# chinaxuyongtao/x264-vs2008

Hardware: AMD Instinct MI355X
Metric: encoded frames/sec, 1080p, preset=medium's flag set with the encoder's own lookahead and rate control (--crf 23 --b-adapt 1, hex, subme 7 RD, trellis 1, psy-rd, aq-mode 1, CABAC payload on the GPU); 1/2/4/8 MI355X (bit-exact) (higher is better)
Workload: dtype u8

## Files before the change

### x264_vs2008_amd/csrc/slice_kernel.h

```cpp
#pragma once
#include <cstddef>
#include <cstring>
#include "me_exact.h"
#include "intra_pred.h"
#include "frame_internal.h"
#include "mb_vocab.h"
#include "trellis_wave.h"
#include "cabac_price.h"

using namespace x264hip;

#define SW_MAX_REFS 8
#define SW_SPIN_LIMIT (1 << 21)
#define SW_MB_BYTES_MAX 8192
#define FD 32
#define FDY (2 * FD)
#define FDU (19 * FD)
#define FDV (19 * FD + 16)

enum { NB_LEFT = 1, NB_TOP = 2, NB_TOPRIGHT = 4, NB_TOPLEFT = 8 };

struct SwRefs {
    const u8 *y[SW_MAX_REFS][4];
    const u8 *u[SW_MAX_REFS], *v[SW_MAX_REFS];
    int ref_bits[SW_MAX_REFS], poc_delta[SW_MAX_REFS], l0_inv_ref_poc[SW_MAX_REFS];
    const u8 *y1[4], *u1, *v1;
    int biw[SW_MAX_REFS];
    int dsf[SW_MAX_REFS], map_col[SW_MAX_REFS];
};
struct SwArgs {
    int mb_w, mb_h, sy, sc, batch, batch_pad;
    int chain;
    size_t bs_y, bs_c;
    int slice_type, qp, qpc, lambda, chroma_skip_thresh, n_refs;
    int l0_n_ref0;
    int me_method, me_range, subme, chroma_me, fast_pskip, dct_decimate, cabac, mv_range;
    int flags_inter, mixed_refs;
    int flags_intra;
    int transform8x8;
    const u16 *q4mf, *q4bias, *q8mf, *q8bias;
    const int *dq4, *dq8;
    const i16 *cost_mv;
    int cost_center;
    const i16 *lowres0, *lowres1;
    const u8 *fy, *fu, *fv;
    u8 *dy, *du, *dv;
    const signed char *l0_type, *l0_ref;
    const i16 *l0_mv;
    signed char *mb_type, *partition, *sub_partition, *ref, *i4mode, *i16mode, *chroma_mode, *qp_out, *t8;
    i16 *mv, *mvr, *cbp;
    u8 *nnz;
    i16 *luma, *luma_dc, *chroma_dc, *chroma_ac;
    int *cost_intra, *cost_inter, *cost_alt;
    int *progress, *abort_flag;
    int *abort_total;
    int spin_limit;
    long long *prof;
    int nr;
    int lossless;
    u32 *nr_sum, *nr_count;
    const u16 *nr_offset;
};

struct SwQp { int qp, qpc, lambda, lambda2, skip_thresh; };

struct SwLds {
    __attribute__((aligned(16))) u8 fe[384];
    u8 fd[27 * FD];
    i16 coef[16][16];
    i16 ccoef[8][16];
    int score[16], cscore[8];
    i16 cdc[8], cdcout[8], dc16[16];
    int keep8, cmode[2], nzdc16;
    i16 lv_y[256], lv_dc[16], lv_cdc[8], lv_cac[128];
    u8 nnz[32];
    i16 mvc[9][2];
    i16 left_mvr[SW_MAX_REFS][2];
    signed char i4c[48];
    u8 e4[16], edge8[40];
    __attribute__((aligned(4))) u8 pt4[48];
    __attribute__((aligned(4))) u8 pt8[80];
    u32 p4lut[48], p8lut[192];
    u16 nr_off4[16], nr_off8[64];
    __attribute__((aligned(16))) u8 patch[MX_PATCH_BYTES];
    u8 i4_fdec[256], i8_fdec[256], i4_nnz[16], i8_nnz[16];
    i16 lv_y8[256];
    i16 t8[256];
    signed char left_i4[4];
    signed char pred4[16], pred8[4];
    i16 l0mvc[SW_MAX_REFS][5][2];
    i16 mv4[16][2];
    signed char ref8[4];
    i16 left_mv4[4][2];
    signed char left_r8[2];
    u16 q8mf[2][64], q8bias[2][64];
    int q8dq[2][64];
    u16 qmf[4][16], qbias[4][16];
    int qdq[4][16];
    i16 costl[2 * MX_COST_LDS + 2];
};

struct SwRd {
    int on;
    int mbrd, trellis, psy_rd;
    int write, cabac_init_idc, i_frame, i_frame_stride;
    int aq, qp_min, qp_max, chroma_qp_offset;
    float f_qpm;
    int psy_trellis;
    const float *aq_offset;
    const i16 *cost_mv_all;
    const int *unq4, *unq8;
    u8 *payload; int payload_cap;
    u32 psy_carry_lo;
    int *payload_len, *mb_bits;
    i16 *mvd;
    i16 *mv1, *mvr1, *mvd1;
    signed char *ref1;
    union {
        u8 *skipbp;
        u8 *mb_carry;
    };
    const signed char *col_type, *col_ref;
    const i16 *col_mv;
    int direct_temporal;
    u32 psy_carry_hi;
    int *direct_score;
    i16 *stale;
};
static_assert(offsetof(SwRd, psy_carry_lo) == offsetof(SwRd, payload_cap) + 4 && offsetof(SwRd, payload_len) == offsetof(SwRd, psy_carry_lo) + 4 &&
              offsetof(SwRd, psy_carry_hi) == offsetof(SwRd, direct_temporal) + 4 && offsetof(SwRd, direct_score) == offsetof(SwRd, psy_carry_hi) + 4,
              "the two halves of the psy-trellis carry's address fill padding: the kernel argument of every other kernel keeps its layout");
struct SwLdsB {
    signed char cref1[48], cskip[48];
    i16 cmv1[48][2], cmvd1[48][2];
    signed char dref[2][4], sub[4];
    i16 dmv[2][16][2];
    i16 mv4_1[16][2];
    signed char ref8_1[4];
    i16 left_mv4_1[4][2], left_mvd1[4][2], left_mvr1[2];
    signed char left_r8_1[2];
    u8 left_skipbp;
    i16 stale[6];
    int me[2][9][6];
    int cost8direct[4];
};
struct SwLdsRdB;
static __device__ const u8 c_bidir_dirs[32] = {149, 21, 101, 69, 89, 81, 86, 84, 165, 5, 105, 65, 90, 80, 150, 20, 153, 17, 102, 68, 133, 37, 97, 73, 88, 82, 22, 148, 145, 25, 100, 70};
struct SwLdsRd {
    u8 cabac[460], cabac_tmp[460];
    signed char cref[48], sub[4];
    i16 cmv[48][2], cmvd[48][2];
    u8 nz_l[4], nz_t[4], nz_lc[2][2], nz_tc[2][2];
    i16 i4_dct[256], i8_dct[256];
    int fenc_satd[16], fenc_sa8d[4];
    int unq4[4][16], unq8[2][64];
    i16 left_mvd[4][2];
    u8 left_nz[8];
    u8 zz2[4], zz4[16], zz8[64];
    int w4z[16], w8z[64];
    u8 zero16[16];
    int tmp_i[4];
    TdWave tw;
};
struct SwLdsNone { int unused; };
struct SwLdsRdB { SwLdsRd r; SwLdsB b; };
struct SwLdsRf { int i16dir[8], cdir[4], i8dir[12][4]; u8 pels[16]; };
struct SwLdsRdF { SwLdsRd r; SwLdsRf f; };
struct MbSynDev {
    int slice_type, type, partition, i16mode, chroma_mode, cbp_luma, cbp_chroma, t8, qp, n_ref, pps_t8, t8_allowed;
    int type_left, type_top, cbp_left, cbp_top, cpm_left, cpm_top, nb_t8, last_qp, last_dqp, prev_coded;
    signed char *sub, *i4c, *cref;
    i16 (*cmv)[2], (*cmvd)[2];
    int n_ref1;
    signed char *cref1, *cskip;
    i16 (*cmv1)[2], (*cmvd1)[2];
    u8 *nnz, *nz_l, *nz_t;
    u8 (*nz_lc)[2], (*nz_tc)[2];
    i16 (*lv4)[16], (*lv8)[64], *lv_dc, (*lv_cdc)[4], (*lv_cac)[16];
};
struct SwTq { static constexpr bool PSY = false; int on; SwLdsRd *r; };
enum { SW_PSY_OWN = 0, SW_PSY_ZERO = 1, SW_PSY_KEPT = 2 };
struct SwTqPsy { static constexpr bool PSY = true; int on; SwLdsRd *r; int psy, src4, src8; i16 *kept; };
__device__ __forceinline__ void sw_tq_set_psy(SwTq &, int, int, i16 *) {}
__device__ __forceinline__ void sw_tq_set_psy(SwTqPsy &tq, int psy, int src, i16 *kept) { tq.psy = psy; tq.src4 = tq.src8 = src; tq.kept = kept; }
__device__ __forceinline__ i16 *sw_psy_carry(const SwRd &rd, int bz)
{
    const unsigned long long p = ((unsigned long long)rd.psy_carry_hi << 32) | rd.psy_carry_lo;
    return p ? (i16 *)p + (size_t)bz * 512 : nullptr;
}
static __device__ const int d_w4z[16] = {800, 320, 320, 800, 128, 800, 320, 320, 320, 320, 128, 800, 128, 320, 320, 128};
static __device__ const u8 d_zz4[16] = {0, 4, 1, 2, 5, 8, 12, 9, 6, 3, 7, 10, 13, 14, 11, 15};
static __device__ const u8 d_zz2[4] = {0, 1, 2, 3};
static __device__ const u16 d_w8k[6] = {256, 201, 656, 227, 410, 363};
static __device__ const u8 d_w8cls[16] = {0, 3, 4, 3, 3, 1, 5, 1, 4, 5, 2, 5, 3, 1, 5, 1};
__device__ __forceinline__ int sw_w8z(int pos) { const int r = c_scan8[0][pos]; return d_w8k[d_w8cls[((r >> 1) & 12) | (r & 3)]]; }
struct SwW8 { __device__ __forceinline__ int operator[](int pos) const { return sw_w8z(pos); } };

#define WAVE_SYNC() do { __builtin_amdgcn_fence(__ATOMIC_RELEASE, "workgroup", "local"); __builtin_amdgcn_wave_barrier(); \
                         __builtin_amdgcn_fence(__ATOMIC_ACQUIRE, "workgroup", "local"); } while (0)

__device__ __forceinline__ void sw_blk_xy(int k, int &x, int &y)
{
    x = ((k >> 2) & 1) * 8 + (k & 1) * 4;
    y = (k >> 3) * 8 + ((k >> 1) & 1) * 4;
}
__device__ __forceinline__ int sw_decimate(const i16 *lv, int n)
{
    int i = n - 1, score = 0;
    while (i >= 0 && lv[i] == 0) i--;
    while (i >= 0) {
        if ((unsigned)(lv[i--] + 1) > 2u) return 9;
        int run = 0;
        while (i >= 0 && lv[i] == 0) { i--; run++; }
        score += c_decimate4[run];
    }
    return score;
}
__device__ __forceinline__ int sw_ue_size(int v) { return v == 0 ? 1 : v < 3 ? 3 : 5; }

__device__ __forceinline__ void sw_mc16(SwLds &s, const SwRefs &refs, const SwArgs &a, int ri, int mvx, int mvy, ptrdiff_t oy, ptrdiff_t oc,
                                        size_t by, size_t bc, int lane, bool do_chroma)
{
    {
        const int r = lane >> 2, x = (lane & 3) * 4;
        const int qx = mvx & 3, qy = mvy & 3, idx = qy * 4 + qx;
        const ptrdiff_t base = oy + (ptrdiff_t)((mvy >> 2) + r) * a.sy + (mvx >> 2) + x + (ptrdiff_t)by;
        const u8 *pa = refs.y[ri][c_qpel_a[idx]] + base + (qy == 3) * a.sy;
        const u8 *pb = refs.y[ri][c_qpel_b[idx]] + base + (qx == 3);
#pragma unroll
        for (int i = 0; i < 4; i++)
            s.fd[FDY + r * FD + x + i] = (idx & 5) ? (u8)(((int)pa[i] + (int)pb[i] + 1) >> 1) : pa[i];
    }
    if (do_chroma) {
        const int cx = lane & 7, cy = lane >> 3;
        const int dx = mvx & 7, dyy = mvy & 7;
        const int ca = (8 - dx) * (8 - dyy), cb = dx * (8 - dyy), cc = (8 - dx) * dyy, cd = dx * dyy;
        const ptrdiff_t cbase = oc + (ptrdiff_t)((mvy >> 3) + cy) * a.sc + (mvx >> 3) + cx + (ptrdiff_t)bc;
        const u8 *pu = refs.u[ri] + cbase, *pv = refs.v[ri] + cbase;
        s.fd[FDU + cy * FD + cx] = (u8)((ca * pu[0] + cb * pu[1] + cc * pu[a.sc] + cd * pu[a.sc + 1] + 32) >> 6);
        s.fd[FDV + cy * FD + cx] = (u8)((ca * pv[0] + cb * pv[1] + cc * pv[a.sc] + cd * pv[a.sc + 1] + 32) >> 6);
    }
}

__device__ __forceinline__ void sw_mc_parts(SwLds &s, const SwRefs &refs, const SwArgs &a, ptrdiff_t oy, ptrdiff_t oc, size_t by, size_t bc, int lane,
                                            bool clip = false, int mbx = 0, int mby = 0)
// ... 1094 lines not shown
```

### x264_vs2008_amd/csrc/slice_sweep_body.h

```cpp
    static_assert(!CH || RD, "the chain table belongs to the raster variant");
    constexpr bool SUB8 = RF && !LL;
    SwRd rd_l;
    if constexpr (CH) {
        typedef const __attribute__((address_space(4))) SwDesc *desc_p;
        const desc_p d = (desc_p)(uintptr_t)tab + blockIdx.x;
        typedef const __attribute__((address_space(4))) u32 *word_p;
        static_assert(sizeof(SwArgs) % 4 == 0 && sizeof(SwRd) % 4 == 0 && alignof(SwDesc) >= 4, "copied by dwords");
        const word_p wa = (word_p)&d->a, wr = (word_p)&d->r;
#pragma unroll
        for (unsigned i = 0; i < sizeof(SwArgs) / 4; i++) ((u32 *)&a)[i] = wa[i];
#pragma unroll
        for (unsigned i = 0; i < sizeof(SwRd) / 4; i++) ((u32 *)&rd_l)[i] = wr[i];
    }
    const SwRd &rd = CH ? rd_l : rd_k;
    const SwRefs &refs = CH ? tab[blockIdx.x].t : refs_k;
    if constexpr (CH && !BS) __builtin_amdgcn_s_setprio(3);
    static_assert(!BS || RD, "B slices run in the raster variant");
    static_assert(!TD || BS, "temporal direct prediction is a B-slice matter");
    static_assert(!RF || (RD && !BS), "the RD refinement is built for the raster variant's I / P kernel");
#undef IS_SKIP_T
#define IS_SKIP_T(t) (BS ? ((t) == T_P_SKIP || (t) == T_B_SKIP) : (t) == T_P_SKIP)
    __builtin_assume(a.lossless == (int)LL);
    __shared__ SwLds s;
    __shared__ typename std::conditional<BS, SwLdsRdB, typename std::conditional<RF, SwLdsRdF, typename std::conditional<RD, SwLdsRd, SwLdsNone>::type>::type>::type sr_;
// ... 491 lines not shown
                } else
                cbp_luma = t8 ? sw_encode_inter_luma8(s, a, Q, tq, lane, &nr_acc8, nr_on) : sw_encode_inter_luma(s, a, Q, tq, lane, &nr_acc4, nr_on);
                cbp_chroma = sw_encode_chroma(s, a, Q, tq, 1, lane);
                if (type == T_P_L0 && part == D_16x16 && !(cbp_luma | cbp_chroma) && mvx == pskx && mvy == psky && ref == 0) type = T_P_SKIP;
                if (BS && type == T_B_DIRECT && !(cbp_luma | cbp_chroma)) type = T_B_SKIP;
            }
        };

        int fenc_satd_sum = 0, fenc_sa8d_sum = 0;
        auto cache_fenc_satd = [&]() {
            if constexpr (PT && !BS) { if (rd.trellis == 2 && a.subme == 6) sw_psy_before_trials(s, tq, a.transform8x8, lane); }
            if (!rd.psy_rd) return;
            int v4 = 0, v8 = 0;
            if (lane < 16) {
                const u8 *fe = s.fe + (lane >> 2) * 64 + (lane & 3) * 4;
                int sad = 0;
#pragma unroll
                for (int j = 0; j < 4; j++)
#pragma unroll
                    for (int i = 0; i < 4; i++) sad += fe[j * 16 + i];
                v4 = satd_4x4(sr.zero16, 0, fe, 16) - (sad >> 1);
            } else if (lane < 20) {
                const int b = lane - 16;
                const u8 *fe = s.fe + (b >> 1) * 128 + (b & 1) * 8;
                int sad = 0;
                for (int j = 0; j < 8; j++)
#pragma unroll
                    for (int i = 0; i < 8; i++) sad += fe[j * 16 + i];
                v8 = ((sa8d_8x8_raw(sr.zero16, 0, fe, 16) + 2) >> 2) - (sad >> 2);
            }
            fenc_satd_sum = wave_sum(v4); fenc_sa8d_sum = wave_sum(v8);
            if constexpr (RF) {
                if (lane < 16) sr.fenc_satd[lane] = v4; else if (lane < 20) sr.fenc_sa8d[lane - 16] = v8;
                WAVE_SYNC();
            }
        };
        auto ssd_mb = [&]() -> int {
            int acc = 0;
            {
                const int r = lane >> 2, x = (lane & 3) * 4, cx = lane & 7, cy = lane >> 3;
#pragma unroll
                for (int i = 0; i < 4; i++) { const int d = (int)s.fe[r * 16 + x + i] - (int)s.fd[FDY + r * FD + x + i]; acc += d * d; }
                const int du = (int)s.fe[256 + cy * 8 + cx] - (int)s.fd[FDU + cy * FD + cx], dv = (int)s.fe[320 + cy * 8 + cx] - (int)s.fd[FDV + cy * FD + cx];
                acc += du * du + dv * dv;
            }
            int ssd = wave_sum(acc);
            if (rd.psy_rd) {
                unsigned long long h = 0;
                if (lane < 4) h = hadamard_ac_8x8(s.fd + FDY + (lane >> 1) * 8 * FD + (lane & 1) * 8, FD);
                const u32 lo = (u32)h, hi = (u32)(h >> 32);
                unsigned long long sum = 0;
#pragma unroll
                for (int k = 0; k < 4; k++) sum += ((unsigned long long)(u32)__builtin_amdgcn_readlane((int)hi, k) << 32) + (u32)__builtin_amdgcn_readlane((int)lo, k);
                const int s4 = (int)((u32)sum >> 1), s8 = (int)(sum >> 34);
                const int satd = (iabs(s4 - fenc_satd_sum) + iabs(s8 - fenc_sa8d_sum)) >> 1;
                ssd += (satd * rd.psy_rd * Q.lambda + 128) >> 8;
            }
            return ssd;
        };
        auto syn_prepare = [&]() {
            if (is_p && lane < 16) {
                const int k = 12 + (lane & 3) + 8 * (lane >> 2);
                sr.cref[k] = s.ref8[(lane >> 3) * 2 + ((lane & 3) >> 1)]; sr.cmv[k][0] = s.mv4[lane][0]; sr.cmv[k][1] = s.mv4[lane][1];
            }
            if (lane < 4) sr.sub[lane] = (signed char)sub_t_mb;
            WAVE_SYNC();
        };
        auto make_syn = [&]() -> MbSynDev {
            MbSynDev y;
            y.slice_type = a.slice_type; y.type = type; y.partition = part; y.i16mode = pred16; y.chroma_mode = predc;
            y.cbp_luma = cbp_luma; y.cbp_chroma = cbp_chroma; y.t8 = t8; y.qp = Q.qp; y.n_ref = a.n_refs; y.pps_t8 = a.transform8x8;
            y.t8_allowed = a.transform8x8 && (type == T_P_L0 || (type == T_P_8x8 && __ballot(lane < 4 && sub_t_mb != D_L0_8x8) == 0));
            if constexpr (BS) y.t8_allowed = a.transform8x8 && type >= T_B_DIRECT && type <= T_B_8x8;
            y.type_left = left_type == T_I_8x8 ? T_I_4x4 : left_type; y.type_top = type_top == T_I_8x8 ? T_I_4x4 : type_top; y.cbp_left = left_cbp; y.cbp_top = cbp_top; y.cpm_left = left_cpm; y.cpm_top = cpm_top;
            y.nb_t8 = (left_type >= 0 && left_t8) + (type_top >= 0 && t8_top);
            y.last_qp = last_qp; y.last_dqp = last_dqp; y.prev_coded = prev_coded;
            y.sub = sr.sub; y.i4c = s.i4c; y.cref = sr.cref; y.cmv = sr.cmv; y.cmvd = sr.cmvd;
            y.n_ref1 = 0; y.cref1 = nullptr; y.cskip = nullptr; y.cmv1 = nullptr; y.cmvd1 = nullptr;
            if constexpr (BS) { y.n_ref1 = 1; y.sub = sb.sub; y.cref1 = sb.cref1; y.cskip = sb.cskip; y.cmv1 = sb.cmv1; y.cmvd1 = sb.cmvd1; }
            y.nnz = s.nnz; y.nz_l = sr.nz_l; y.nz_t = sr.nz_t; y.nz_lc = sr.nz_lc; y.nz_tc = sr.nz_tc;
            y.lv4 = (i16 (*)[16])s.lv_y; y.lv8 = (i16 (*)[64])s.lv_y8; y.lv_dc = s.lv_dc; y.lv_cdc = (i16 (*)[4])s.lv_cdc; y.lv_cac = (i16 (*)[16])s.lv_cac;
            return y;
        };
        auto price_mb = [&]() -> int {
            syn_prepare();
            for (int k = lane; k < 460; k += 64) sr.cabac_tmp[k] = sr.cabac[k];
            const MbSynDev y0 = make_syn();
            const CpMasks km = cp_masks([&](int q) -> cp_u64 { return __ballot(cp_mask_lane(y0, q, lane)); });
            WAVE_SYNC();
            if (lane == 0) {
                DCabac tcb = {0, 0x1FE, -1, 0, nullptr, 0};
                MbSynDev y = y0;
                cp_macroblock(tcb, sr.cabac_tmp, y, km);
                sr.tmp_i[0] = tcb.f8;
            }
            WAVE_SYNC();
            return UNI(sr.tmp_i[0]);
        };
        (void)cache_fenc_satd; (void)ssd_mb; (void)price_mb;
        const int satd_pcm = RD && !rd.psy_rd && mbrd ? (int)(((unsigned long long)(386 * 8) * (u32)Q.lambda2 + 128) >> 8) : MX_COST_MAX;

        if constexpr (BS) {
#include "slice_b_flow.h"
        } else
        if (!RD && !is_p) {
          {
            analyse_intra(MX_COST_MAX);
            type = T_I_16x16;
            int i_cost = satd_i16;
            if (satd_i4 < i_cost) { i_cost = satd_i4; type = T_I_4x4; }
            if (satd_i8 < i_cost) { i_cost = satd_i8; type = T_I_8x8; }
          }
        } else {
            int ra = left_ref, ax = left_mvx, ay = left_mvy;
            int rb = -2, bx = 0, byv = 0, rc = -2, cx = 0, cy = 0;
            if (is_p && (nb & NB_TOP)) { const int o = mb - a.mb_w; rb = UNI(a.ref[o * 4 + 2]); bx = UNI(a.mv[(o * 16 + 12) * 2]); byv = UNI(a.mv[(o * 16 + 12) * 2 + 1]); }
            if (!is_p) {}
            else if (nb & NB_TOPRIGHT) { const int o = mb - a.mb_w + 1; rc = UNI(a.ref[o * 4 + 2]); cx = UNI(a.mv[(o * 16 + 12) * 2]); cy = UNI(a.mv[(o * 16 + 12) * 2 + 1]); }
            else if (nb & NB_TOPLEFT) { const int o = mb - a.mb_w - 1; rc = UNI(a.ref[o * 4 + 3]); cx = UNI(a.mv[(o * 16 + 15) * 2]); cy = UNI(a.mv[(o * 16 + 15) * 2 + 1]); }
            int cref_v = -2, cmvx_v = 0, cmvy_v = 0, pme_v = 0;
            int sub_mx = 0, sub_my = 0, sub_cost = 0, sub_px = 0, sub_py = 0, sub_t = D_L0_8x8;
            int sub_cst = MX_COST_MAX;
            (void)sub_cst;
            if (is_p && (RD || (a.flags_inter & 0x10))) {
                if ((nb & NB_TOP) && lane >= 4 && lane < 8) {
                    const int o = mb - a.mb_w, k = lane - 4;
                    cref_v = a.ref[o * 4 + 2 + (k >> 1)]; cmvx_v = a.mv[(o * 16 + 12 + k) * 2]; cmvy_v = a.mv[(o * 16 + 12 + k) * 2 + 1];
                }
                if ((nb & NB_TOPLEFT) && lane == 3) {
                    const int o = mb - a.mb_w - 1;
                    cref_v = a.ref[o * 4 + 3]; cmvx_v = a.mv[(o * 16 + 15) * 2]; cmvy_v = a.mv[(o * 16 + 15) * 2 + 1];
                }
                if ((nb & NB_TOPRIGHT) && lane == 8) {
                    const int o = mb - a.mb_w + 1;
                    cref_v = a.ref[o * 4 + 2]; cmvx_v = a.mv[(o * 16 + 12) * 2]; cmvy_v = a.mv[(o * 16 + 12) * 2 + 1];
                }
                if ((nb & NB_LEFT) && lane >= 11 && lane < 36 && ((lane - 11) & 7) == 0) {
                    const int i = (lane - 11) >> 3;
                    cref_v = s.left_r8[i >> 1]; cmvx_v = s.left_mv4[i][0]; cmvy_v = s.left_mv4[i][1];
                }
            }
            if constexpr (RD) { if (is_p && lane == 30) { cref_v = st0r; cmvx_v = st0x; cmvy_v = st0y; } }
            if constexpr (RD) {
                if (is_p) {
                    if (lane < 48) { sr.cref[lane] = (signed char)cref_v; sr.cmv[lane][0] = (i16)cmvx_v; sr.cmv[lane][1] = (i16)cmvy_v; }
                    WAVE_SYNC();
                }
            }
            auto predict16 = [&](int i_ref, int &px, int &py) {
                const int cnt = (ra == i_ref) + (rb == i_ref) + (rc == i_ref);
                if (cnt > 1) { px = mb_median(ax, bx, cx); py = mb_median(ay, byv, cy); }
                else if (cnt == 1) { if (ra == i_ref) { px = ax; py = ay; } else if (rb == i_ref) { px = bx; py = byv; } else { px = cx; py = cy; } }
                else if (rb == -2 && rc == -2 && ra != -2) { px = ax; py = ay; }
                else { px = mb_median(ax, bx, cx); py = mb_median(ay, byv, cy); }
            };
            if (ra == -2 || rb == -2 || !(ra | ax | ay) || !(rb | bx | byv)) { pskx = 0; psky = 0; }
            else predict16(0, pskx, psky);

            int b_skip = 0, try_pskip = 0;
            if (is_p && a.fast_pskip) {
                if (a.subme >= 3) try_pskip = 1;
                else if (left_type == T_P_SKIP || type_top == T_P_SKIP || type_topleft == T_P_SKIP || type_topright == T_P_SKIP) {
                    b_skip = sw_probe_pskip(s, refs, a, Q, pskx, psky, mbx, mby, oy, oc, by_, bc_, lane);
                    skip_mc = b_skip;
                }
            }
            if (b_skip) type = T_P_SKIP;
            else {
                const MeLimits L = me_limits(mbx, mby, a.mb_w, a.mb_h, a.mv_range);
                MxCtx c;
                c.fe = (MX_LDS(u32))s.fe; c.fe_u = (MX_LDS(u8))(s.fe + 256); c.fe_v = (MX_LDS(u8))(s.fe + 320); c.sy = a.sy; c.sc = a.sc; c.lane = lane; c.set_block(16, 16, 0, 0);
                c.cost_g = (MX_GLB(i16))cost_g;
                c.cost_l = (MX_LDS(i16))s.costl; c.has_cost_l = true; c.patch = (MX_LDS(u8))s.patch; c.has_patch = true; c.patch_on = false;
                int thresh = 0x7fffffff, best = 0x7fffffff, bmvpx = 0, bmvpy = 0;
                bool early_skip = false;
                for (int r = 0; r < (is_p ? a.n_refs : 0); r++) {
// ... 468 lines not shown
                                    continue;
                                } else {
                                    tq.on = rd.trellis != 0;
                                    if (rd.trellis == 1 || a.nr) skip_intra = 0;
                                }
                            } else if (step == 11) {
                                if constexpr (RF) {
#include "slice_refine.h"
                                }
                            } else {
                                fin = true;
                                tq.on = rd.trellis != 0;
                                if (rd.trellis == 1 || a.nr) skip_intra = 0;
                            }
                            if ((!fin || mbrd) && !IS_INTRA_T(type)) update_cache_p();
                            const int t8_bak = t8;
                            PROF(6);
                            if (!(fin && type == T_I_PCM)) encode_mb(fin ? 1 : 0);
                            else psy_after_analysis();
                            if (fin) { encoded = true; break; }
                            PROF(0);
                            int c = ssd_mb();
                            if (type == T_P_SKIP) c += (Q.lambda2 + 128) >> 8;
                            else {
                                const int f8 = price_mb();
                                c += (int)(((unsigned long long)(u32)f8 * (u32)Q.lambda2 + 32768) >> 16);
                            }
                            t8 = t8_bak;
                            PROF(7);
                            if (step == 0) { rd16 = c; if (type == T_P_SKIP) rd_skip = true; }
                            else if (step == 2) rd16 = c;
                            else if (step == 3) c16x8 = c;
                            else if (step == 4) c8x16 = c;
                            else if (step == 5) c8x8 = c;
                            else if (step == 6) {
                                if (i_cost >= c) {
                                    if (i_cost > 0) satd_inter = (int)((long long)satd_inter * c / i_cost);
                                    if (satd_inter == 0) satd_inter = 1;
                                    i_cost = c;
                                } else
                                    t8 = !t8;
                            } else if (step == 7) satd_i16 = c;
                            else if (step == 8) satd_i4 = c;
                            else if (step == 9) { satd_i8 = c; i8_cbp_rd = cbp_luma; }
                            else if constexpr (RF) {
                                if (rf_kind == 1) { if ((unsigned long long)(u32)c < rf_best) { rf_best = (unsigned long long)(u32)c; rf_best16 = pred16; } }
                                else {
                                    type = T_P_L0;
                                    if ((unsigned long long)(u32)c < rf_best) { rf_best = (unsigned long long)(u32)c; q_bmx = q_cx; q_bmy = q_cy; if (q_tag != -3) q_dir = q_tag; }
                                }
                                step = 10;
                            }
                        }
                    }
                }
            }
            if constexpr (RD) {
                if (is_p && rd.stale) {
                    if (type == T_P_SKIP) { st0r = 0; st0x = pskx; st0y = psky; }
                    else if (!IS_INTRA_T(type) && encoded) { st0r = UNI(s.ref8[3]); st0x = UNI(s.mv4[10][0]); st0y = UNI(s.mv4[10][1]); }
                    else { st0r = __builtin_amdgcn_readlane(cref_v, 30); st0x = __builtin_amdgcn_readlane(cmvx_v, 30); st0y = __builtin_amdgcn_readlane(cmvy_v, 30); }
                }
            }
        }
        (void)analysed;
        if constexpr (!RD) PROF(6);
        LAUNDER();

        if constexpr (!RD) encode_mb(1);
        else if (!encoded) encode_pskip();
        const int intra = IS_INTRA_T(type);
        int mb_qp = Q.qp, cbp_store = 0;
        if constexpr (RD) {
            PROF(3);
            if (type == T_I_PCM) {
                *(u32 *)(s.fd + FDY + (lane >> 2) * FD + (lane & 3) * 4) = *(const u32 *)(s.fe + (lane >> 2) * 16 + (lane & 3) * 4);
                s.fd[FDU + (lane >> 3) * FD + (lane & 7)] = s.fe[256 + lane]; s.fd[FDV + (lane >> 3) * FD + (lane & 7)] = s.fe[320 + lane];
                cbp_luma = 0xf; cbp_chroma = 2; t8 = 0;
                WAVE_SYNC();
            }
            if (rd.write) {
                syn_prepare();
                const MbSynDev y0 = make_syn();
                if (lane == 0) {
                    if (mb > 0) cd_encode_terminal(cab);
                    if (IS_SKIP_T(type)) cw_mb_skip(cab, sr.cabac, left_type, type_top, 1, a.slice_type);
                    else {
                        if (is_p || BS) cw_mb_skip(cab, sr.cabac, left_type, type_top, 0, a.slice_type);
                        MbSynDev y = y0;
                        cw_macroblock(cab, sr.cabac, 0, y, s.fe, rd.i_frame + bz * rd.i_frame_stride);
                        sr.tmp_i[1] = y.qp;
                    }
                    const int pos = cd_pos(cab, payload0);
                    if (rd.mb_bits) rd.mb_bits[cb + mb] = pos;
                    sr.tmp_i[2] = (pos >> 3) + SW_MB_BYTES_MAX + 64 > rd.payload_cap;
                }
                WAVE_SYNC();
                if (UNI(sr.tmp_i[2])) {
                    if (lane == 0) { __hip_atomic_store(a.abort_flag, 1, __ATOMIC_RELAXED, __HIP_MEMORY_SCOPE_AGENT); atomicAdd(a.abort_total, 1); }
                    return;
                }
                if (!IS_SKIP_T(type)) mb_qp = UNI(sr.tmp_i[1]);
            } else if (type == T_I_16x16 && !(cbp_luma | cbp_chroma) && !UNI((int)s.nnz[24])) {
                mb_qp = last_qp;
            }
            if (SUB8 && type == T_I_PCM) {
                mb_qp = 0; last_dqp = 0; if (lane == 24) s.nnz[24] = 0; WAVE_SYNC();
            } else
            if (type == T_I_PCM) { mb_qp = 0; last_dqp = 0; if (lane < 27) s.nnz[lane] = 16; WAVE_SYNC(); }
            else {
                if (type != T_I_16x16 && cbp_luma == 0 && cbp_chroma == 0) mb_qp = last_qp;
                last_dqp = mb_qp - last_qp; last_qp = mb_qp;
            }
        }
        if (cbp_luma == 0 && type != T_I_8x8) t8 = 0;
        PROF(RD ? 5 : 3);
        LAUNDER();

        {
            const int r = lane >> 2, x = (lane & 3) * 4;
            *(u32 *)(a.dy + oy + (ptrdiff_t)r * a.sy + x) = *(const u32 *)(s.fd + FDY + r * FD + x);
            if (lane < 32) {
                const int chn = lane >> 4, l = lane & 15, cr = l >> 1, cx4 = (l & 1) * 4;
                *(u32 *)((chn ? a.dv : a.du) + oc + (ptrdiff_t)cr * a.sc + cx4) = *(const u32 *)(s.fd + (chn ? FDV : FDU) + cr * FD + cx4);
            }
        }
        if (lane < 16) {
            a.mv[((size_t)mb * 16 + lane) * 2] = (i16)(intra ? 0 : s.mv4[lane][0]);
            a.mv[((size_t)mb * 16 + lane) * 2 + 1] = (i16)(intra ? 0 : s.mv4[lane][1]);
            if ((lane & 3) == 3) { s.left_mv4[lane >> 2][0] = (i16)(intra ? 0 : s.mv4[lane][0]); s.left_mv4[lane >> 2][1] = (i16)(intra ? 0 : s.mv4[lane][1]); }
            const bool i48 = type == T_I_4x4 || type == T_I_8x8;
            a.i4mode[(size_t)mb * 16 + lane] = i48 ? s.i4c[mb_scan8_luma(lane)] : (signed char)2;
            if (lane == 5 || lane == 7 || lane == 13 || lane == 15)
                s.left_i4[lane == 5 ? 0 : lane == 7 ? 1 : lane == 13 ? 2 : 3] = i48 ? s.i4c[mb_scan8_luma(lane)] : (signed char)2;
        }
        if (lane < 4) {
            const signed char rv = (signed char)(is_p || BS ? (intra ? -1 : s.ref8[lane]) : -1);
            a.ref[(size_t)mb * 4 + lane] = rv;
            if (lane & 1) s.left_r8[lane >> 1] = rv;
        }
        if (lane < 27) (a.nnz + 27 * cb)[(size_t)mb * 27 + lane] = IS_SKIP_T(type) ? (u8)0 : SUB8 && type == T_I_PCM ? (u8)16 : s.nnz[lane];
        if (lane < 4) (a.sub_partition + 4 * cb)[(size_t)mb * 4 + lane] = (signed char)(type == T_P_8x8 ? sub_t_mb : BS && type == T_B_8x8 ? (int)sb.sub[lane] : 0);
        if constexpr (BS) {
            if (lane < 16) {
                const i16 vx = (i16)(intra ? 0 : sb.mv4_1[lane][0]), vy = (i16)(intra ? 0 : sb.mv4_1[lane][1]);
                (rd.mv1 + 32 * cb)[((size_t)mb * 16 + lane) * 2] = vx; (rd.mv1 + 32 * cb)[((size_t)mb * 16 + lane) * 2 + 1] = vy;
                if ((lane & 3) == 3) { sb.left_mv4_1[lane >> 2][0] = vx; sb.left_mv4_1[lane >> 2][1] = vy; }
            }
            if (lane < 4) {
                const signed char rv1 = (signed char)(intra ? -1 : sb.ref8_1[lane]);
                (rd.ref1 + 4 * cb)[(size_t)mb * 4 + lane] = rv1;
                if (lane & 1) sb.left_r8_1[lane >> 1] = rv1;
            }
            if (lane == 0) {
                const int sbp = type == T_B_SKIP || type == T_B_DIRECT ? 0xf
                              : type == T_B_8x8 ? (sb.sub[0] == D_DIRECT_8x8) | (sb.sub[1] == D_DIRECT_8x8) << 1 | (sb.sub[2] == D_DIRECT_8x8) << 2 | (sb.sub[3] == D_DIRECT_8x8) << 3 : 0;
                (rd.skipbp + cb)[mb] = (u8)sbp; sb.left_skipbp = (u8)sbp;
            }
        }
        if (lane == 0) {
            const int cbp_dc = a.cabac ? (s.nnz[24] | s.nnz[25] << 1 | s.nnz[26] << 2) : 0;
            a.mb_type[mb] = (signed char)type;
            (a.partition + cb)[mb] = (signed char)(intra || IS_SKIP_T(type) || (BS && type == T_B_DIRECT) ? D_16x16 : part);
            (a.i16mode + cb)[mb] = (signed char)(type == T_I_16x16 ? pred16 : 0);
            (a.chroma_mode + cb)[mb] = (signed char)(intra ? predc : 0);
            (a.qp_out + cb)[mb] = (signed char)mb_qp;
            (a.t8 + cb)[mb] = (signed char)t8;
            (a.cbp + cb)[mb] = (i16)(IS_SKIP_T(type) ? 0 : type == T_I_PCM ? 0x72f : (cbp_dc << 8) | (cbp_chroma << 4) | cbp_luma);
            (a.cost_intra + cb)[mb] = stat_intra; (a.cost_inter + cb)[mb] = stat_inter; (a.cost_alt + cb)[mb] = stat_alt;
        }
        if (a.luma) {
            const bool coded = !IS_SKIP_T(type) && type != T_I_PCM;
            i16 *ly = (a.luma + 256 * cb) + (size_t)mb * 256, *cac = (a.chroma_ac + 128 * cb) + (size_t)mb * 128;
// ... 82 lines not shown
```

Measured before the change: 481.5.

## Precompute CABAC coded-block flags and significance masks wave-wide before serial lane-0 coding

Adds a CABAC residual coder that consumes per-block coded_block_flag contexts and significance bitmasks computed in parallel by all lanes (ballots and per-lane cbf context). Both the RD bit-pricing trials and the final bitstream writer use it, so the serial lane-0 loop no longer derives neighbour contexts or scans coefficients for zeros. The writer stores its masks in the idle cabac_tmp buffer and adds an extra wave sync, and a small cbf array is added to LDS. Which kernel variants take the new path is decided by compile-time macros, and the output must stay bit-exact.

```diff
diff --git a/x264_vs2008_amd/csrc/cabac_resolved.h b/x264_vs2008_amd/csrc/cabac_resolved.h
--- /dev/null
+++ b/x264_vs2008_amd/csrc/cabac_resolved.h
@@ -0,0 +1,99 @@
+#pragma once
+#include "cabac_price.h"
+
+#define CR_CBF_N 27
+template <class MS> CD_FN int cr_cbf_lane(const MS &m, int lane)
+{
+    const int cat = lane < 16 ? (m.type == T_I_16x16 ? 1 : 2) : lane < 24 ? 4 : lane == 24 ? 0 : 3;
+    return (85 + cw_cbf_ctx(m, cat, lane)) | (m.nnz[lane] ? 0x80 : 0);
+}
+
+template <int RD, class ST, class LV> CD_FN void cr_residual(DCabac &cb, ST st, int cat, LV l, int count, cp_u64 mask, int cbf)
+{
+    const int c_sig = CD_SIG_OFF(cat), c_last = CD_LAST_OFF(cat), c_lvl = CD_LEVEL_OFF(cat), b8 = cat == 5;
+    if (!b8) {
+        if (!(cbf & 0x80)) { cdd(cb, st, RD, cbf, 0); return; }
+        cdd(cb, st, RD, cbf & 0x7f, 1);
+    }
+    if (!mask) return;
+    const int last = 63 - __builtin_clzll(mask);
+    int node = 0;
+    if constexpr (!RD) {
+        const int sigmap = last + 1 < count - 1 ? last + 1 : count - 1;
+        for (int i = 0; i < sigmap; i++) {
+            const int cs = c_sig + (b8 ? CP_UNI(CD_SIG8(i)) : i), cl = c_last + (b8 ? CP_UNI(CD_LAST8(i)) : i);
+            if ((mask >> i) & 1) { cd_encode_decision(cb, st, cs, 1); cd_encode_decision(cb, st, cl, i == last); }
+            else cd_encode_decision(cb, st, cs, 0);
+        }
+        for (cp_u64 rest = mask; rest;) {
+            const int i = 63 - __builtin_clzll(rest);
+            rest ^= 1ull << i;
+            const int v = CP_UNI(l[i]);
+            const int am1 = cd_abs(v) - 1, prefix = am1 < 14 ? am1 : 14;
+            int ctx = CD_LVL1_CTX(node) + c_lvl;
+            if (prefix) {
+                cd_encode_decision(cb, st, ctx, 1);
+                ctx = CD_LVLGT1_CTX(node) + c_lvl;
+                for (int k = 0; k < prefix - 1; k++) cd_encode_decision(cb, st, ctx, 1);
+                if (prefix < 14) cd_encode_decision(cb, st, ctx, 0);
+                else cd_encode_ue_bypass(cb, 0, am1 - 14);
+                node = CD_NODE_NEXT1(node);
+            } else {
+                cd_encode_decision(cb, st, ctx, 0);
+                node = CD_NODE_NEXT0(node);
+            }
+            cd_encode_bypass(cb, v < 0);
+        }
+    } else {
+        for (int i = last; i >= 0; i--) {
+            const int cs = c_sig + (b8 ? CP_UNI(CD_SIG8(i < 63 ? i : 62)) : i), cl = c_last + (b8 ? CP_UNI(CD_LAST8(i < 63 ? i : 62)) : i);
+            if (i == last) {
+                if (last != count - 1) { cdd(cb, st, 1, cs, 1); cdd(cb, st, 1, cl, 1); }
+            } else if ((mask >> i) & 1) { cdd(cb, st, 1, cs, 1); cdd(cb, st, 1, cl, 0); }
+            else { cdd(cb, st, 1, cs, 0); continue; }
+            const int v = CP_UNI(l[i]);
+            const int am1 = cd_abs(v) - 1, prefix = am1 < 14 ? am1 : 14;
+            int ctx = CD_LVL1_CTX(node) + c_lvl;
+            if (prefix) {
+                cdd(cb, st, 1, ctx, 1);
+                ctx = CD_LVLGT1_CTX(node) + c_lvl;
+                cb.f8 += cd_unary(st, ctx, prefix);
+                if (prefix >= 14) cd_ue(cb, 1, 0, am1 - 14);
+                node = CD_NODE_NEXT1(node);
+            } else {
+                cdd(cb, st, 1, ctx, 0);
+                node = CD_NODE_NEXT0(node);
+                cb.f8 += 256;
+            }
+        }
+    }
+}
+
+#define CR_MASK_WORDS 14
+struct CrMaskRegs { const CpMasks &k; };
+template <class W> struct CrMaskWords { W w; };
+CD_FN cp_u64 cr_mask(const CrMaskRegs &s, int cat, int idx) { return cp_block_mask(s.k, cat, idx); }
+template <class W> CD_FN cp_u64 cr_mask(const CrMaskWords<W> &s, int cat, int idx)
+{
+    const int q = cat == 0 || cat == 3 ? 6 : cat == 4 ? 4 + (idx >= 20) : idx >> 2;
+    const cp_u64 v = (cp_u64)(u32)CP_UNI(s.w[2 * q]) | ((cp_u64)(u32)CP_UNI(s.w[2 * q + 1]) << 32);
+    const CpMasks k = {v, v, v, v, v, v, v};
+    return cp_block_mask(k, cat, idx);
+}
+
+template <int RD, class ST, class MS, class FE, class MK, class CB> CD_FN void cr_macroblock(DCabac &cb, ST st, MS &m, FE fe, int i_frame, const MK &mk, CB cbf)
+{
+    const int type = m.type;
+    if (!cw_mb_head(cb, st, RD, m, fe, i_frame)) return;
+#define CR_BLOCK(cat_, idx_, l_, n_) cr_residual<RD>(cb, st, cat_, l_, n_, cr_mask(mk, cat_, idx_), (cat_) == 5 ? 0 : CP_UNI(cbf[idx_]))
+    if (type == T_I_16x16) {
+        CR_BLOCK(0, 24, &m.lv_dc[0], 16);
+        if (m.cbp_luma) for (int i = 0; i < 16; i++) CR_BLOCK(1, i, &m.lv4[i][1], 15);
+    } else if (m.t8) {
+        for (int i = 0; i < 4; i++) if (m.cbp_luma & (1 << i)) CR_BLOCK(5, 4 * i, &m.lv8[i][0], 64);
+    } else
+        for (int i = 0; i < 16; i++) if (m.cbp_luma & (1 << (i >> 2))) CR_BLOCK(2, i, &m.lv4[i][0], 16);
+    if (m.cbp_chroma & 3) { CR_BLOCK(3, 25, &m.lv_cdc[0][0], 4); CR_BLOCK(3, 26, &m.lv_cdc[1][0], 4); }
+    if (m.cbp_chroma & 2) for (int i = 16; i < 24; i++) CR_BLOCK(4, i, &m.lv_cac[i - 16][1], 15);
+#undef CR_BLOCK
+}
diff --git a/x264_vs2008_amd/csrc/slice_kernel.h b/x264_vs2008_amd/csrc/slice_kernel.h
--- a/x264_vs2008_amd/csrc/slice_kernel.h
+++ b/x264_vs2008_amd/csrc/slice_kernel.h
@@ -6,7 +6,13 @@
 #include "frame_internal.h"
 #include "mb_vocab.h"
 #include "trellis_wave.h"
-#include "cabac_price.h"
+#include "cabac_resolved.h"
+#ifndef SW_CR_TRIALS
+#define SW_CR_TRIALS (!LL && (PT || BS || RF || !CH))
+#endif
+#ifndef SW_CR_WRITER
+#define SW_CR_WRITER (!LL && (PT || BS || RF || !CH))
+#endif
 
 using namespace x264hip;
 
@@ -161,6 +167,7 @@
     u8 zero16[16];
     int tmp_i[4];
     TdWave tw;
+    u8 cbf[28];
 };
 struct SwLdsNone { int unused; };
 struct SwLdsRdB { SwLdsRd r; SwLdsB b; };
diff --git a/x264_vs2008_amd/csrc/slice_sweep_body.h b/x264_vs2008_amd/csrc/slice_sweep_body.h
--- a/x264_vs2008_amd/csrc/slice_sweep_body.h
+++ b/x264_vs2008_amd/csrc/slice_sweep_body.h
@@ -597,16 +597,19 @@
             y.lv4 = (i16 (*)[16])s.lv_y; y.lv8 = (i16 (*)[64])s.lv_y8; y.lv_dc = s.lv_dc; y.lv_cdc = (i16 (*)[4])s.lv_cdc; y.lv_cac = (i16 (*)[16])s.lv_cac;
             return y;
         };
+        constexpr bool cr_trials = SW_CR_TRIALS, cr_writer = SW_CR_WRITER;
         auto price_mb = [&]() -> int {
             syn_prepare();
             for (int k = lane; k < 460; k += 64) sr.cabac_tmp[k] = sr.cabac[k];
             const MbSynDev y0 = make_syn();
             const CpMasks km = cp_masks([&](int q) -> cp_u64 { return __ballot(cp_mask_lane(y0, q, lane)); });
+            if constexpr (cr_trials) { if (lane < CR_CBF_N) sr.cbf[lane] = (u8)cr_cbf_lane(y0, lane); }
             WAVE_SYNC();
             if (lane == 0) {
                 DCabac tcb = {0, 0x1FE, -1, 0, nullptr, 0};
                 MbSynDev y = y0;
-                cp_macroblock(tcb, sr.cabac_tmp, y, km);
+                if constexpr (cr_trials) cr_macroblock<1>(tcb, sr.cabac_tmp, y, (const u8 *)nullptr, 0, CrMaskRegs{km}, sr.cbf);
+                else cp_macroblock(tcb, sr.cabac_tmp, y, km);
                 sr.tmp_i[0] = tcb.f8;
             }
             WAVE_SYNC();
@@ -1241,13 +1244,24 @@
             if (rd.write) {
                 syn_prepare();
                 const MbSynDev y0 = make_syn();
+                u32 *const wmask = (u32 *)sr.cabac_tmp;
+                static_assert(offsetof(SwLdsRd, cabac_tmp) % 4 == 0 && CR_MASK_WORDS * 4 <= sizeof(sr.cabac_tmp), "the writer's masks fit the idle copy of the contexts");
+                if (cr_writer && !IS_SKIP_T(type)) {
+                    for (int q = 0; q < CR_MASK_WORDS / 2; q++) {
+                        const cp_u64 b = __ballot(cp_mask_lane(y0, q, lane));
+                        if (lane == 0) { wmask[2 * q] = (u32)b; wmask[2 * q + 1] = (u32)(b >> 32); }
+                    }
+                    if (lane < CR_CBF_N) sr.cbf[lane] = (u8)cr_cbf_lane(y0, lane);
+                }
+                if constexpr (cr_writer) WAVE_SYNC();
                 if (lane == 0) {
                     if (mb > 0) cd_encode_terminal(cab);
                     if (IS_SKIP_T(type)) cw_mb_skip(cab, sr.cabac, left_type, type_top, 1, a.slice_type);
                     else {
                         if (is_p || BS) cw_mb_skip(cab, sr.cabac, left_type, type_top, 0, a.slice_type);
                         MbSynDev y = y0;
-                        cw_macroblock(cab, sr.cabac, 0, y, s.fe, rd.i_frame + bz * rd.i_frame_stride);
+                        if constexpr (cr_writer) cr_macroblock<0>(cab, sr.cabac, y, s.fe, rd.i_frame + bz * rd.i_frame_stride, CrMaskWords<const u32 *>{wmask}, sr.cbf);
+                        else cw_macroblock(cab, sr.cabac, 0, y, s.fe, rd.i_frame + bz * rd.i_frame_stride);
                         sr.tmp_i[1] = y.qp;
                     }
                     const int pos = cd_pos(cab, payload0);
```

After: 484.2, median of 3. About the same (+0.6%).
